# ClashLuke/LocAtE

Hardware: AMD Instinct MI355X
Metric: images/sec (G+D step) 64x64 bs=64 (higher is better)
Workload: dtype f32 (contractions fp32-faithful on the matrix cores: 2 x scaled fp16 operand pieces / 3 MFMAs per slice where the operand's largest magnitude comes with it, else 3 x bf16 pieces / 6 MFMAs; fp32 accumulate); 1 GPU; LocAtE G+D step, 64x64 RGB, batch 64 per GPU (the fp32 variant - the reference's own precision - of BASELINE.json configs[1]: 64x64 RGB bs 64), self/feature attention at 16x16 and 64x64, random-init weights; global_batch=64, image_size=64, parallelism=dp1, launch=hipGraph replay, G-step generator pass on a second stream

## Files before the change

locate_amd/build.py:

```python
import os
import shutil
import subprocess
import sys

CSRC = os.path.join(os.path.dirname(os.path.abspath(__file__)), "csrc")
LIB = os.path.join(CSRC, "liblocate_hip.so")
LIB_DBG = os.path.join(CSRC, "liblocate_hip_dbg.so")
DBG_SOURCES = ["conv.hip", "convwgrad.hip", "convwin.hip", "snapshot.hip"]
SOURCES = ["runtime.hip", "elementwise.hip", "norm.hip", "softmax.hip", "resample.hip", "spectral.hip", "conv.hip", "convpack.hip", "convwgrad.hip", "convwin.hip", "convfp8.hip",
           "grouped.hip", "nadam.hip", "loss.hip", "finalise.hip", "parallel.hip", "input.hip", "grid.hip", "swd.hip", "average.hip", "stats.hip", "guard.hip", "snapshot.hip", "digest.hip", "dynamics.hip", "neighbours.hip", "formats.hip", "spectrum.hip", "msssim.hip", "modes.hip"]
ARCH = "gfx950"


def _hipcc():
    for cand in (os.environ.get("HIPCC"), shutil.which("hipcc"), "/opt/rocm/bin/hipcc"):
        if cand and os.path.exists(cand):
            return cand
    raise RuntimeError("hipcc not found: the MI355X kernels cannot be built")


def _sources():
    return [s for s in SOURCES if os.path.exists(os.path.join(CSRC, s))]


def _headers():
    return [os.path.join(CSRC, h) for h in sorted(os.listdir(CSRC)) if h.endswith(".h")]


def needs_build():
    if not (os.path.exists(LIB) and os.path.exists(LIB_DBG)):
        return True
    t = min(os.path.getmtime(LIB), os.path.getmtime(LIB_DBG))
    deps = [os.path.join(CSRC, s) for s in _sources()] + _headers()
    return any(os.path.getmtime(d) > t for d in deps)


def build(force=False, verbose=True):
    if not force and not needs_build():
        return LIB
    hipcc = _hipcc()
    objs = []
    flags = ["--offload-arch=" + ARCH, "-O3", "-fPIC", "-std=c++17", "-fvisibility=hidden", "-Wall", "-Wno-unused-function",
             "-I", CSRC]
    procs = []
    hdr_time = max(os.path.getmtime(h) for h in _headers())
    for src in _sources():
        path = os.path.join(CSRC, src)
        obj = os.path.join(CSRC, src.replace(".hip", ".o"))
        objs.append(obj)
        if not force and os.path.exists(obj) and os.path.getmtime(obj) > max(os.path.getmtime(path), hdr_time):
            continue
        cmd = [hipcc] + flags + ["-c", path, "-o", obj]
        if verbose:
            print(" ".join(cmd), flush=True)
        procs.append((src, subprocess.Popen(cmd)))
    dbg_objs = list(objs)
    for src in DBG_SOURCES:
        path = os.path.join(CSRC, src)
        obj = os.path.join(CSRC, src.replace(".hip", "_dbg.o"))
        dbg_objs[dbg_objs.index(os.path.join(CSRC, src.replace(".hip", ".o")))] = obj
        if not force and os.path.exists(obj) and os.path.getmtime(obj) > max(os.path.getmtime(path), hdr_time):
            continue
        cmd = [hipcc] + flags + ["-DLOCATE_DEBUG_KNOBS", "-c", path, "-o", obj]
        if verbose:
            print(" ".join(cmd), flush=True)
        procs.append((src + " (debug)", subprocess.Popen(cmd)))
    failed = [src for src, p in procs if p.wait() != 0]
    if failed:
        raise RuntimeError("hipcc failed on " + ", ".join(failed))
    cmd = [hipcc, "--offload-arch=" + ARCH, "-shared", "-fPIC", "-o", LIB] + objs
    if verbose:
        print(" ".join(cmd), flush=True)
    subprocess.check_call(cmd)
    subprocess.check_call([hipcc, "--offload-arch=" + ARCH, "-shared", "-fPIC", "-o", LIB_DBG] + dbg_objs)
    return LIB


if __name__ == "__main__":
    build(force="--force" in sys.argv)
    print(LIB)
```

locate_amd/csrc/conv.hip:

```cpp
#include "igemm.h"

template <int WGM, int WGN, int TM, int TN>
__global__ void __launch_bounds__(256) conv_igemm_kernel(const IgParams p) {
    constexpr int BK = IG_BK;
    constexpr int BM = WGM * TM * 32;
    constexpr int BN = WGN * TN * 32;
    constexpr int KPT = BK * BN / 256;
    constexpr int A_F4 = BK * BM / 4;
    constexpr int A_PT = (A_F4 + 255) / 256;
    static_assert(WGM * WGN == 4, "four waves");
    static_assert(BN % 64 == 0 && KPT == 8, "one 8-row group of the offset table per thread and step");
    static_assert(BK <= IG_TAIL, "panel tail shorter than the prefetch distance (one stage beyond the last)");

    __shared__ __attribute__((aligned(16))) float As[2][BK][BM];
    __shared__ __attribute__((aligned(16))) float Bs[2][BK][BN];

    int bx, by, bz;
    xcd_tile(bx, by, bz, p.tile_nphase);
    const int zphase = bz / p.ksplit, zsplit = bz - zphase * p.ksplit;
    const IgPhase& ph = p.ph[zphase];
    const int N = p.B * ph.QH * ph.QW;
    const int n0 = bx * BN;
    const int m0 = by * BM;
    if (n0 >= N) return;
// ... 462 lines not shown
    const float sc = p.scale ? p.scale[(p.scale_bg ? b / p.scale_bg : 0) * p.scale_stride] : 1.0f;
    float* op = p.out + (long long)b * p.out_bs + q;
    if (p.act_out == nullptr && p.mul_pre == nullptr) {
#pragma unroll
        for (int m = 0; m < MT; ++m) {
            if (m < p.M && live) {
                const float bv = p.bias ? p.bias[m] : 0.0f;
                const float v0 = fmaf(acc[m][0], sc, bv), v1 = fmaf(acc[m][PX - 1], sc, bv);
                if (PX == 2) *reinterpret_cast<float2*>(op + (long long)m * HW) = make_float2(v0, v1);
                else op[(long long)m * HW] = v0;
            }
        }
        return;
    }
    float am = 0.0f;
    const float* zp = p.mul_pre ? p.mul_pre + (long long)b * p.mul_bs + q : nullptr;
    float* ap = p.act_out ? p.act_out + (long long)b * p.act_bs + q : nullptr;
#pragma unroll
    for (int m = 0; m < MT; ++m) {
        if (m < p.M && live) {
            const float bv = p.bias ? p.bias[m] : 0.0f;
            float v0 = fmaf(acc[m][0], sc, bv), v1 = fmaf(acc[m][PX - 1], sc, bv);
            if (zp) {
                float z0, z1;
                if (PX == 2) { const float2 t = *reinterpret_cast<const float2*>(zp + (long long)m * HW); z0 = t.x; z1 = t.y; }
                else { z0 = zp[(long long)m * HW]; z1 = z0; }
                v0 = roottanh_grad_f(z0, v0); v1 = roottanh_grad_f(z1, v1);
                am = fmaxf(am, fmaxf(fabsf(v0), fabsf(v1)));
            }
            if (PX == 2) *reinterpret_cast<float2*>(op + (long long)m * HW) = make_float2(v0, v1);
            else op[(long long)m * HW] = v0;
            if (ap) {
                const float a0 = roottanh_f(v0), a1 = roottanh_f(v1);
                if (PX == 2) *reinterpret_cast<float2*>(ap + (long long)m * HW) = make_float2(a0, a1);
                else ap[(long long)m * HW] = a0;
                am = fmaxf(am, fmaxf(fabsf(a0), fabsf(a1)));
            }
        }
    }
    if (p.out_absmax) absmax_publish_wave(am, p.out_absmax);
}


#define SK_NT 4
#define SK_RC 32
#define SK_WAVES 8

__global__ void __launch_bounds__(64 * SK_WAVES) skinny_rows_kernel(const IgParams p) {
    const IgPhase& ph = p.ph[0];
    const int R = ph.K, J = p.M, N = p.B, ld = ph.ld;
    const int lane = threadIdx.x & 63, wid = __builtin_amdgcn_readfirstlane((int)threadIdx.x >> 6);
    const int j = blockIdx.x * 64 + lane;
    const int n0 = blockIdx.y * SK_NT;
    const bool jok = j < ld;
    const float* __restrict__ P = ph.wp + (jok ? j : 0);
    const float* __restrict__ in = p.in;
    float acc[SK_NT];
#pragma unroll
    for (int t = 0; t < SK_NT; ++t) acc[t] = 0.0f;
    const int nchunk = (R + SK_RC - 1) / SK_RC;
    float cur[SK_RC], nxt[SK_RC];
    if (wid < nchunk) {
#pragma unroll
        for (int i = 0; i < SK_RC; ++i) cur[i] = P[(long long)(wid * SK_RC + i) * ld];
    }
    for (int c = wid; c < nchunk; c += SK_WAVES) {
        const int r0 = c * SK_RC;
        if (c + SK_WAVES < nchunk) {
#pragma unroll
            for (int i = 0; i < SK_RC; ++i) nxt[i] = P[(long long)(r0 + SK_WAVES * SK_RC + i) * ld];
        }
        if (r0 + SK_RC <= R) {
#pragma unroll
            for (int t = 0; t < SK_NT; ++t) {
                if (n0 + t < N) {
                    const float* __restrict__ xr = in + (long long)(n0 + t) * p.in_bs + r0;
#pragma unroll
                    for (int i = 0; i < SK_RC; ++i) acc[t] = fmaf(xr[i], cur[i], acc[t]);
                }
            }
        } else {
#pragma unroll
            for (int t = 0; t < SK_NT; ++t) {
                if (n0 + t < N) {
                    const float* __restrict__ xr = in + (long long)(n0 + t) * p.in_bs + r0;
#pragma unroll
                    for (int i = 0; i < SK_RC; ++i) {
                        const float xv = r0 + i < R ? xr[i] : 0.0f;
                        acc[t] = fmaf(xv, cur[i], acc[t]);
                    }
                }
            }
        }
#pragma unroll
        for (int i = 0; i < SK_RC; ++i) cur[i] = nxt[i];
    }
    __shared__ float red[SK_WAVES][SK_NT][64];
#pragma unroll
    for (int t = 0; t < SK_NT; ++t) red[wid][t][lane] = acc[t];
    __syncthreads();
    if (wid < SK_NT) {
        const int n = n0 + wid;
        float am = 0.0f;
        if (n < N && j < J) {
            float s = red[0][wid][lane];
#pragma unroll
            for (int w = 1; w < SK_WAVES; ++w) s += red[w][wid][lane];
            const float sc = p.scale ? p.scale[(p.scale_bg ? n / p.scale_bg : 0) * p.scale_stride] : 1.0f;
            float v = fmaf(s, sc, p.bias ? p.bias[j] : 0.0f);
            if (p.mul_pre) { v = roottanh_grad_f(p.mul_pre[(long long)n * p.mul_bs + j], v); am = fabsf(v); }
            p.out[(long long)n * p.out_bs + j] = v;
            if (p.act_out) { const float a = roottanh_f(v); p.act_out[(long long)n * p.act_bs + j] = a; am = fabsf(a); }
        }
        if (p.out_absmax) absmax_publish_wave(am, p.out_absmax);
        if (p.lat && blockIdx.x == 0 && n < N)
            for (int c = lane; c < p.lat_z; c += 64) p.act_out[(long long)n * p.act_bs - p.lat_z + c] = p.lat[(long long)n * p.lat_bs + c];
    }
}

static bool skinny_ok(const IgParams& p) {
    if (p.nphase != 1 || path_disabled("skinny")) return false;
    const IgPhase& ph = p.ph[0];
    return ph.T == 1 && p.H == 1 && p.W == 1 && p.OH == 1 && p.OW == 1 && ph.dy0 == 0 && ph.dx0 == 0 && ph.K >= 1;
}

static void launch_skinny(const IgParams& p, hipStream_t st) {
    skinny_rows_kernel<<<dim3((p.M + 63) / 64, (p.B + SK_NT - 1) / SK_NT), 64 * SK_WAVES, 0, st>>>(p);
}

static bool pointwise_ok(const IgParams& p) {
    if (p.nphase != 1 || path_disabled("pointwise")) return false;
    const IgPhase& ph = p.ph[0];
    const int HW = p.H * p.W;
    return ph.T == 1 && p.istride == 1 && p.ostep == 1 && ph.dy0 == 0 && ph.dx0 == 0 && p.H == p.OH && p.W == p.OW &&
           ph.K >= 1 && ph.K <= 64 && p.M <= 64 && ph.ld >= ((p.M + 15) / 16) * 16 && (HW & 1) == 0 && (p.in_bs & 1) == 0 &&
           (p.out_bs & 1) == 0 && (reinterpret_cast<uintptr_t>(p.in) & 7) == 0 && (reinterpret_cast<uintptr_t>(p.out) & 7) == 0 &&
           (long long)p.B * HW >= 131072 &&
           (!p.act_out || ((p.act_bs & 1) == 0 && (reinterpret_cast<uintptr_t>(p.act_out) & 7) == 0)) &&
           (!p.mul_pre || ((p.mul_bs & 1) == 0 && (reinterpret_cast<uintptr_t>(p.mul_pre) & 7) == 0));
}

template <int PX>
static void launch_pointwise_px(const IgParams& p, hipStream_t st) {
    const long long npx = (long long)p.B * p.H * p.W / PX;
    const int blocks = (int)((npx + 255) / 256);
    const int mt = (p.M + 15) / 16;
    if (mt == 1) conv_pointwise_kernel<16, PX><<<blocks, 256, 0, st>>>(p);
    else if (mt == 2) conv_pointwise_kernel<32, PX><<<blocks, 256, 0, st>>>(p);
    else if (mt == 3) conv_pointwise_kernel<48, PX><<<blocks, 256, 0, st>>>(p);
    else conv_pointwise_kernel<64, PX><<<blocks, 256, 0, st>>>(p);
}

static void launch_pointwise(const IgParams& p, hipStream_t st) {
    if ((long long)p.B * p.H * p.W >= (long long)knob_int("LOCATE_PX2_MIN", 2 * 256 * 1024)) launch_pointwise_px<2>(p, st);
    else launch_pointwise_px<1>(p, st);
}

static int igemm_bm(int M, int nmax, int nphase) {
    if (M % 192 == 0 && M >= 192 && !path_disabled("tall") && !path_disabled("bx6")) {
        const long long tiles = (long long)((nmax + 127) / 128) * (M / 192) * nphase;
        if (tiles >= 512) return 192;
    }
    return pick_bm(M);
}

static int igemm_ksplit(int M, int nmax, int nphase, int min_kpad) {
    const int bm = igemm_bm(M, nmax, nphase);
    const long long tiles = (long long)((nmax + 127) / 128) * ((M + bm - 1) / bm) * nphase;
    const int slots = bm == 192 ? 512 : 768;
    if (tiles >= slots || (tiles >= 512 && tiles % 256 == 0)) return 1;
    const int steps = min_kpad / IG_BK;
    long long want = (slots + tiles - 1) / tiles;
    const int min_steps = (long long)M * nmax <= (1 << 16) ? 2 : 8;
    if (steps < 8) return 1;
    const int max_split = steps / min_steps > 0 ? steps / min_steps : 1;
    if (want > max_split) want = max_split;
    if (want > 64) want = 64;
    if (want > knob_int("LOCATE_KS_MAX", 64)) want = knob_int("LOCATE_KS_MAX", 64);
    return want < 1 ? 1 : (int)want;
}

#define IG_MAX_COUNTERS 1024
struct SplitPlan {
    int ksplit, combine, gx, gy;
    size_t slab_floats;
};

static SplitPlan igemm_split_plan(const IgParams& p, int nmax, bool have_counters) {
    SplitPlan sp;
    const int bm = igemm_bm(p.M, nmax, p.nphase);
    int min_kpad = 1 << 30;
    for (int i = 0; i < p.nphase; ++i) min_kpad = p.ph[i].Kpad < min_kpad ? p.ph[i].Kpad : min_kpad;
    int ks = igemm_ksplit(p.M, nmax, p.nphase, min_kpad);
    if (ks > min_kpad / IG_BK) ks = min_kpad / IG_BK;
    if (ks < 1) ks = 1;
    sp.ksplit = ks;
    sp.gx = (nmax + 127) / 128;
    sp.gy = (p.M + bm - 1) / bm;
    const long long ntiles = (long long)sp.gx * sp.gy * p.nphase;
    const long long tile_floats = (long long)bm * 128;
    const long long legacy = ks > 1 ? (long long)ks * p.B * p.M * p.OH * p.OW : 0;
    const long long fused = ks > 1 ? (long long)ks * ntiles * tile_floats : 0;
    sp.combine = have_counters && ks > 1 && (long long)ks * tile_floats * 4 <= (512 << 10) && ntiles <= IG_MAX_COUNTERS &&
                 fused * 4 < (1ll << 31) && (p.precision == 1 || !path_disabled("bx6")) && !path_disabled("combine");
    sp.slab_floats = (size_t)(sp.combine ? fused : legacy);
    return sp;
}

void launch_slab_reduce(const IgParams& p, hipStream_t st) {
    igemm_slab_reduce_kernel<<<stream_grid(p.slab_stride, 256), 256, 0, st>>>(p.slab, p.out, p.bias, p.scale, p.scale_bg, p.scale_stride, p.B, p.M, p.OH * p.OW,
                                                                              p.out_bs, p.slab_stride, p.ksplit, p.act_out, p.act_bs, p.mul_pre, p.mul_bs, p.out_absmax);
}

template <int NP>
static void launch_bx6(const IgParams& p, dim3 grid, int bm, bool w8, hipStream_t st) {
    if (w8) {
        if (bm == 128) conv_igemm_bx6_kernel<2, 4, 2, 1, NP, 8><<<grid, 512, 0, st>>>(p);
        else conv_igemm_bx6_kernel<2, 4, 1, 1, NP, 8><<<grid, 512, 0, st>>>(p);
        return;
    }
    with_tile<true>(bm, [&](auto t) { using T = decltype(t); conv_igemm_bx6_kernel<T::wgm, T::wgn, T::tm, T::tn, NP><<<grid, 256, 0, st>>>(p); });
}

static int launch_igemm(IgParams& p, int nmax, void* slab_ws, unsigned* counters, hipStream_t st, const char* who) {
    p.tile_nphase = (path_disabled("phasefast") || (long long)p.OH * p.OW < 1024) ? 1 : p.nphase;
    if (p.win) return launch_win_igemm(p, nmax, slab_ws, counters, st, who);
    if (skinny_ok(p)) {
        p.ksplit = 1;
        launch_skinny(p, st);
        LOCATE_LAUNCH_CHECK(who);
        return LOCATE_OK;
    }
    if (pointwise_ok(p)) {
        p.ksplit = 1;
        launch_pointwise(p, st);
        LOCATE_LAUNCH_CHECK(who);
        return LOCATE_OK;
    }
    const int bm = igemm_bm(p.M, nmax, p.nphase);
    const SplitPlan sp = igemm_split_plan(p, nmax, counters != nullptr);
    p.ksplit = sp.ksplit;
    p.combine = sp.combine;
    p.counters = counters;
    p.slab = static_cast<float*>(slab_ws);
    p.slab_stride = (long long)p.B * p.M * p.OH * p.OW;
    dim3 grid(sp.gx, sp.gy, p.nphase * p.ksplit);
    for (int i = 0; i < p.nphase; ++i)
        LOCATE_REQUIRE(round_up(p.M, bm) <= p.ph[i].ld, "%s: tile height %d does not divide the panel width %d", who, bm, p.ph[i].ld);
    if (p.precision == 3) {
        launch_fp8_igemm(p, grid, bm, st);
        LOCATE_LAUNCH_CHECK(who);
        if (p.ksplit > 1 && !p.combine) {
            LOCATE_REQUIRE(p.slab_stride < (1ll << 31), "%s: split-K output of %lld elements exceeds the 32-bit index range", who, p.slab_stride);
            launch_slab_reduce(p, st);
            LOCATE_LAUNCH_CHECK(who);
        }
        return LOCATE_OK;
    }
    const bool w8 = !path_disabled("w8") && !path_disabled("bx6") && (bm == 128 || bm == 64) &&
                    (long long)grid.x * grid.y * grid.z <= knob_int("LOCATE_W8_MAX", 320);
    if (p.precision == 2) LOCATE_REQUIRE(!path_disabled("bx6"), "%s: fp16 pieces need the bf16/fp16 MFMA kernels", who);
    if (p.precision == 1) launch_bx6<1>(p, grid, bm, w8, st);
    else if (p.precision == 2) launch_bx6<2>(p, grid, bm, w8, st);
    else if (!path_disabled("bx6")) launch_bx6<3>(p, grid, bm, w8, st);
    else with_tile<false>(bm, [&](auto t) { using T = decltype(t); conv_igemm_kernel<T::wgm, T::wgn, T::tm, T::tn><<<grid, 256, 0, st>>>(p); });
    LOCATE_LAUNCH_CHECK(who);
    if (p.ksplit > 1 && !p.combine) {
        const long long total = p.slab_stride;
        LOCATE_REQUIRE(total < (1ll << 31), "%s: split-K output of %lld elements exceeds the 32-bit index range", who, total);
        launch_slab_reduce(p, st);
        LOCATE_LAUNCH_CHECK(who);
    }
    return LOCATE_OK;
}

static size_t slab_floats(const IgParams& p, int nmax) {
    if (p.win) return win_slab_floats(p, nmax);
    if (skinny_ok(p)) return 0;
    const size_t a = igemm_split_plan(p, nmax, false).slab_floats, b = igemm_split_plan(p, nmax, true).slab_floats;
    return a > b ? a : b;
}

static void useful_taps(int in, int out, int k, int s, int pad, int* lo, int* n) {
    if (path_disabled("taps")) { *lo = 0; *n = k; return; }
    int first = -1, last = -1;
    for (int t = 0; t < k; ++t) {
        bool any = false;
        for (int o = 0; o < out && !any; ++o) {
            const int i = o * s - pad + t;
            any = i >= 0 && i < in;
        }
        if (any) { if (first < 0) first = t; last = t; }
    }
    if (first < 0) { first = 0; last = 0; }
    *lo = first; *n = last - first + 1;
}
static void useful_phase_taps(int Q, int out, int d0, int T, int* lo, int* n) {
    if (path_disabled("taps")) { *lo = 0; *n = T > 0 ? T : 1; return; }
    int first = T > 0 ? d0 - out + 1 : 0, last = d0 + Q - 1;
    if (first < 0) first = 0;
    if (last > T - 1) last = T - 1;
    if (first > last) { first = 0; last = 0; }
    *lo = first; *n = last - first + 1;
}

static void phase_taps(int parity, int pad, int K, int s, int* k0, int* d0, int* T) {
// ... 375 lines not shown
```

locate_amd/csrc/igemm.h:

```cpp
#pragma once
#include "common.h"
#include <cstdlib>
#include <cstring>
#include <stdlib.h>
#include <type_traits>

#ifdef LOCATE_DEBUG_KNOBS
static bool path_disabled(const char* name) {
    static const char* env = getenv("LOCATE_DISABLE");
    return env != nullptr && strstr(env, name) != nullptr;
}
static int knob_int(const char* name, int fallback) {
    const char* v = getenv(name);
    return v != nullptr ? atoi(v) : fallback;
}
#else
static constexpr bool path_disabled(const char*) { return false; }
static constexpr int knob_int(const char*, int fallback) { return fallback; }
#endif

typedef float f32x16 __attribute__((ext_vector_type(16)));

#define IG_BK 16
#define IG_KPAD 32
// ... 67 lines not shown
    const unsigned* wmax;
    int direct;
    int keep_f32;
    int win, Tp, urows, wmax_single;
};

#define PACK_MAX_TAPS 32
struct PackBatch {
    PackArgs ph[4];
};
struct PackJob {
    PackBatch batch;
    int nphase, kind;
    int gx, gy;
    int block_start, pad;
};
PackJob make_pack_job(const PackBatch& b, int nphase);
int launch_pack(const PackBatch& b, int nphase, hipStream_t st, const char* who);

#define PANEL_HDR 4
static inline size_t panel_floats(int rows, int ld, int fmt) {
    if (fmt == 2) return (size_t)rows * ld + rows + rows / 4 + PANEL_HDR + (size_t)rows * ld / 4;
    return (size_t)rows * ld + rows + rows / 4 + (fmt ? PANEL_HDR + (size_t)rows * ld / 2 * 2 : (size_t)rows * ld / 2 * 3);
}
static inline size_t panel_split_offset(int rows, int ld) { return (size_t)rows * ld + rows + rows / 4; }
__device__ __forceinline__ size_t panel_split_offset_dev(int rows, int ld) { return (size_t)rows * ld + rows + rows / 4; }

__host__ __device__ __forceinline__ int scale_exp_below(int top, unsigned bits, unsigned grown) {
    const unsigned field = (bits >> 23) & 0xffu;
    if (grown == 0u ? field - 1u >= 254u : field == 255u) return 0;
    const int k = top - ((int)(field + grown) - 127);
    return k > 126 ? 126 : (k < -126 ? -126 : k);
}
__host__ __device__ __forceinline__ int f16_scale_exp(unsigned bits, unsigned grown = 0u) { return scale_exp_below(14, bits, grown); }
__host__ __device__ __forceinline__ int f8_scale_exp(unsigned bits, unsigned grown = 0u) { return scale_exp_below(7, bits, grown); }
__device__ __forceinline__ float pow2f(int k) { return __uint_as_float((unsigned)(k + 127) << 23); }
__device__ __forceinline__ void unscale_pair(int ka, int kb, float& u1, float& u2) {
    const int t = -(ka + kb), h = t >> 1;
    u1 = pow2f(h);
    u2 = pow2f(t - h);
}

typedef __bf16 bf16x8 __attribute__((ext_vector_type(8)));

__device__ __forceinline__ void split3_bf16x8(const float (&v)[8], bf16x8& h, bf16x8& m, bf16x8& l) {
#pragma unroll
    for (int j = 0; j < 8; ++j) {
        h[j] = (__bf16)v[j];
        const float r1 = v[j] - (float)h[j];
        m[j] = (__bf16)r1;
        l[j] = (__bf16)(r1 - (float)m[j]);
    }
}

__device__ __forceinline__ void split3_trunc_pair(float v0, float v1, unsigned& h, unsigned& m, unsigned& l) {
    const unsigned u0 = __builtin_bit_cast(unsigned, v0), u1 = __builtin_bit_cast(unsigned, v1);
    const float r0 = v0 - __builtin_bit_cast(float, u0 & 0xffff0000u), r1 = v1 - __builtin_bit_cast(float, u1 & 0xffff0000u);
    const unsigned q0 = __builtin_bit_cast(unsigned, r0), q1 = __builtin_bit_cast(unsigned, r1);
    const float l0 = r0 - __builtin_bit_cast(float, q0 & 0xffff0000u), l1 = r1 - __builtin_bit_cast(float, q1 & 0xffff0000u);
    h = __builtin_amdgcn_perm(u1, u0, 0x07060302u);
    m = __builtin_amdgcn_perm(q1, q0, 0x07060302u);
    l = __builtin_amdgcn_perm(__builtin_bit_cast(unsigned, l1), __builtin_bit_cast(unsigned, l0), 0x07060302u);
}

__device__ __forceinline__ unsigned round_bf16_pair(float v0, float v1) {
    typedef __bf16 bf16x2_t __attribute__((ext_vector_type(2)));
    bf16x2_t r;
    r[0] = (__bf16)v0;
    r[1] = (__bf16)v1;
    return *reinterpret_cast<unsigned*>(&r);
}

__device__ __forceinline__ void split3_trunc_x8(const float (&v)[8], uint4& h, uint4& m, uint4& l) {
    split3_trunc_pair(v[0], v[1], h.x, m.x, l.x);
    split3_trunc_pair(v[2], v[3], h.y, m.y, l.y);
    split3_trunc_pair(v[4], v[5], h.z, m.z, l.z);
    split3_trunc_pair(v[6], v[7], h.w, m.w, l.w);
}

typedef _Float16 f16x8 __attribute__((ext_vector_type(8)));

__device__ __forceinline__ void split2_f16x8(const float (&v)[8], float sc, uint4& h, uint4& l) {
    f16x8 hh, ll;
#pragma unroll
    for (int j = 0; j < 8; ++j) {
        const float x = v[j] * sc;
        hh[j] = (_Float16)x;
        ll[j] = (_Float16)(x - (float)hh[j]);
    }
    h = *reinterpret_cast<uint4*>(&hh);
    l = *reinterpret_cast<uint4*>(&ll);
}

__device__ __forceinline__ void split2_f16_pair(float v0, float v1, unsigned& h, unsigned& l) {
    typedef _Float16 f16x2 __attribute__((ext_vector_type(2)));
    f16x2 hh, ll;
    hh[0] = (_Float16)v0; hh[1] = (_Float16)v1;
    ll[0] = (_Float16)(v0 - (float)hh[0]); ll[1] = (_Float16)(v1 - (float)hh[1]);
    h = *reinterpret_cast<unsigned*>(&hh);
    l = *reinterpret_cast<unsigned*>(&ll);
}

struct IgPhase {
    const float* wp;
    const int* koff;
    const unsigned char* ktap;
    const uint4* w3;
    const unsigned* a_absmax;
    long long w3_plane;
    int K, Kpad, ld, T;
    int dmin;
    int oy0, ox0, QH, QW;
    int TW, tw_magic;
    int dy0, dys, dx0, dxs;
    int win_Tp, win_NG, win_TR, win_NI, win_WR;
    unsigned win_wrw_mul;
    int win_wrw_s1, win_wrw_s2;
    int tapc[32] __attribute__((aligned(32)));
};

struct IgParams {
    const float* in;
    float* out;
    const float* bias;
    const float* scale;
    int scale_bg;
    int scale_stride;
    long long in_bs, out_bs;
    unsigned in_bytes;
    int B, C, H, W;
    int M, OH, OW;
    int istride, ostep, nphase;
    int ksplit;
    float* slab;
    long long slab_stride;
    int precision;
    const unsigned* b_absmax;
    float* act_out = nullptr;
    long long act_bs = 0;
    const float* lat = nullptr;
    long long lat_bs = 0;
    int lat_z = 0;
    const float* mul_pre = nullptr;
    long long mul_bs = 0;
    unsigned* out_absmax = nullptr;
    int combine;
    unsigned* counters;
    int tile_nphase;
    int win;
    int win_dbg;
    int win_U, win_slotsp, win_bm, win_bn;
    IgPhase ph[4];
};

template <int WGM, int WGN, int TM, int TN>
__device__ __forceinline__ void igemm_col_scales(const IgParams& p, const IgPhase& ph, float (&col_scale)[TN], int N, int n0,
                                                 int wn, int lane) {
    const int lcol = lane & 31;
#pragma unroll
    for (int j = 0; j < TN; ++j) {
        const int nj = n0 + (wn * TN + j) * 32 + lcol;
        const int nn = nj < N ? nj : 0;
        const int b = nn / (ph.QH * ph.QW);
        col_scale[j] = p.scale ? p.scale[(p.scale_bg ? b / p.scale_bg : 0) * p.scale_stride] : 1.0f;
    }
}

template <int WGM, int WGN, int TM, int TN>
__device__ __forceinline__ void igemm_epilogue(const IgParams& p, const IgPhase& ph, f32x16 (&acc)[TM][TN],
                                               const float (&col_scale)[TN], int N, int n0, int m0, int zsplit, int wm,
                                               int wn, int lane, float* stage, bool split) {
    const int lrow = lane >> 5, lcol = lane & 31;
    const long long plane = (long long)p.OH * p.OW;
    const int iplane = (int)plane;
    if (stage != nullptr && p.nphase == 1 && p.ostep == 1 && iplane <= 16 && (iplane & (iplane - 1)) == 0 &&
        ph.QH * ph.QW == iplane) {
        const int lp = __ffs(iplane) - 1;
        const bool fused_s = !split && (p.act_out != nullptr || p.mul_pre != nullptr);
        float am_s = 0.0f;
        float* out_base = split ? p.slab + (long long)zsplit * p.slab_stride : p.out;
        const long long obs = split ? (long long)p.M * plane : p.out_bs;
#pragma unroll
        for (int i = 0; i < TM; ++i) {
            const int mt0 = m0 + (wm * TM + i) * 32;
            float bias_v[16];
#pragma unroll
            for (int r = 0; r < 16; ++r) {
                const int m = mt0 + (r & 3) + 8 * (r >> 2) + 4 * lrow;
                const bool use = p.bias != nullptr && !split && m < p.M;
                const float* bp = use ? p.bias + m : p.in;
                bias_v[r] = use ? *bp : 0.0f;
            }
#pragma unroll
            for (int j = 0; j < TN; ++j) {
                const int nt0 = n0 + (wn * TN + j) * 32;
#pragma unroll
                for (int r = 0; r < 16; ++r) {
                    const int ml = (r & 3) + 8 * (r >> 2) + 4 * lrow;
                    stage[lcol * 33 + ml] = split ? acc[i][j][r] : fmaf(acc[i][j][r], col_scale[j], bias_v[r]);
                }
                __builtin_amdgcn_fence(__ATOMIC_SEQ_CST, "wavefront");
                const int b0 = nt0 >> lp;
                if (!fused_s) {
#pragma unroll
                    for (int e = 0; e < 16; ++e) {
                        const int flat = e * 64 + lane;
                        const int bl = flat >> (5 + lp), rem = flat & ((32 << lp) - 1);
                        const int ml = rem >> lp, pix = rem & (iplane - 1);
                        const int nl = (bl << lp) + pix;
                        const float v = stage[nl * 33 + ml];
                        if (nt0 + nl < N && mt0 + ml < p.M) out_base[(long long)(b0 + bl) * obs + (long long)(mt0 + ml) * plane + pix] = v;
                    }
                } else if (WGM * WGN == 8 && TM * TN <= 2 && p.mul_pre != nullptr) {
                    __builtin_amdgcn_sched_barrier(0);
                    float z[16];
#pragma unroll
                    for (int e = 0; e < 16; ++e) {
                        const int flat = e * 64 + lane;
                        const int bl = flat >> (5 + lp), rem = flat & ((32 << lp) - 1);
                        const int ml = rem >> lp, pix = rem & (iplane - 1);
                        const int nl = (bl << lp) + pix;
                        const bool ok = nt0 + nl < N && mt0 + ml < p.M;
                        z[e] = ok ? p.mul_pre[(long long)(b0 + bl) * p.mul_bs + (long long)(mt0 + ml) * plane + pix] : 0.0f;
                    }
#pragma unroll
                    for (int e = 0; e < 16; ++e) {
                        const int flat = e * 64 + lane;
                        const int bl = flat >> (5 + lp), rem = flat & ((32 << lp) - 1);
                        const int ml = rem >> lp, pix = rem & (iplane - 1);
                        const int nl = (bl << lp) + pix;
                        if (nt0 + nl < N && mt0 + ml < p.M) {
                            const float v = roottanh_grad_f(z[e], stage[nl * 33 + ml]);
                            am_s = fmaxf(am_s, fabsf(v));
                            out_base[(long long)(b0 + bl) * obs + (long long)(mt0 + ml) * plane + pix] = v;
                        }
                    }
                    __builtin_amdgcn_sched_barrier(0);
                } else {
#pragma unroll 1
                    for (int e = 0; e < 16; ++e) {
                        const int flat = e * 64 + lane;
                        const int bl = flat >> (5 + lp), rem = flat & ((32 << lp) - 1);
                        const int ml = rem >> lp, pix = rem & (iplane - 1);
                        const int nl = (bl << lp) + pix;
                        float v = stage[nl * 33 + ml];
                        if (nt0 + nl < N && mt0 + ml < p.M) {
                            const long long rel = (long long)(mt0 + ml) * plane + pix;
                            if (p.mul_pre != nullptr) {
                                v = roottanh_grad_f(p.mul_pre[(long long)(b0 + bl) * p.mul_bs + rel], v);
                                am_s = fmaxf(am_s, fabsf(v));
                            }
                            out_base[(long long)(b0 + bl) * obs + rel] = v;
                            if (p.mul_pre == nullptr) {
                                const float a = roottanh_f(v);
                                p.act_out[(long long)(b0 + bl) * p.act_bs + rel] = a;
                                am_s = fmaxf(am_s, fabsf(a));
                            }
                        }
                    }
                }
                __builtin_amdgcn_fence(__ATOMIC_SEQ_CST, "wavefront");
            }
        }
        if (fused_s && p.out_absmax != nullptr) absmax_publish_wave(am_s, p.out_absmax);
        return;
    }
    const float* optr[TN];
    long long xoff[TN];
    const bool fused = !split && (p.act_out != nullptr || p.mul_pre != nullptr);
#pragma unroll
    for (int j = 0; j < TN; ++j) {
        const int nj = n0 + (wn * TN + j) * 32 + lcol;
        const int nn = nj < N ? nj : 0;
        const int qhw = ph.QH * ph.QW;
        const int b = nn / qhw, q = nn - b * qhw;
        const int qy = q / ph.QW, qx = q - qy * ph.QW;
        const long long pix = (long long)(ph.oy0 + qy * p.ostep) * p.OW + (ph.ox0 + qx * p.ostep);
        const float* o = split ? p.slab + (long long)zsplit * p.slab_stride + (long long)b * p.M * plane + pix
                               : p.out + (long long)b * p.out_bs + pix;
        optr[j] = nj < N ? o : nullptr;
        xoff[j] = (long long)b * ((p.mul_pre ? p.mul_bs : p.act_bs) - p.out_bs);
    }
    float am = 0.0f;
#pragma unroll
    for (int i = 0; i < TM; ++i) {
        float bias_v[16];
#pragma unroll
        for (int r = 0; r < 16; ++r) {
            const int m = m0 + (wm * TM + i) * 32 + (r & 3) + 8 * (r >> 2) + 4 * lrow;
            const bool use = p.bias != nullptr && !split && m < p.M;
            const float* bp = use ? p.bias + m : p.in;
            bias_v[r] = use ? *bp : 0.0f;
        }
#pragma unroll
        for (int j = 0; j < TN; ++j) {
            float* o = const_cast<float*>(optr[j]);
            if (o == nullptr) continue;
            if (!fused) {
#pragma unroll
                for (int r = 0; r < 16; ++r) {
                    const int m = m0 + (wm * TM + i) * 32 + (r & 3) + 8 * (r >> 2) + 4 * lrow;
                    if (m < p.M) o[(long long)m * plane] = split ? acc[i][j][r] : fmaf(acc[i][j][r], col_scale[j], bias_v[r]);
                }
            } else if (p.mul_pre != nullptr) {
                const float* pre = p.mul_pre + ((o - p.out) + xoff[j]);
#pragma unroll
// ... 115 lines not shown
```

Before: 7368 images/sec.

## Add MFMA-based persistent pointwise conv kernel with register-resident weights

Adds a new 1x1 (pointwise) convolution kernel that keeps the weights in registers and computes on fp32 32x32x2 MFMA instructions. It runs as a persistent grid capped at a per-CU block count, with a ring buffer that prefetches the next tile's input while the current tile computes. It can also fuse the roottanh activation, its gradient multiply and absmax publishing into the epilogue. It replaces the scalar pointwise kernel when shapes and alignment qualify, aiming to lift arithmetic throughput and hide load latency, at the cost of many templated variants and heavy register pressure.

```diff
diff --git a/locate_amd/build.py b/locate_amd/build.py
--- a/locate_amd/build.py
+++ b/locate_amd/build.py
@@ -7,7 +7,7 @@
 LIB = os.path.join(CSRC, "liblocate_hip.so")
 LIB_DBG = os.path.join(CSRC, "liblocate_hip_dbg.so")
 DBG_SOURCES = ["conv.hip", "convwgrad.hip", "convwin.hip", "snapshot.hip"]
-SOURCES = ["runtime.hip", "elementwise.hip", "norm.hip", "softmax.hip", "resample.hip", "spectral.hip", "conv.hip", "convpack.hip", "convwgrad.hip", "convwin.hip", "convfp8.hip",
+SOURCES = ["runtime.hip", "elementwise.hip", "norm.hip", "softmax.hip", "resample.hip", "spectral.hip", "conv.hip", "convpw.hip", "convpack.hip", "convwgrad.hip", "convwin.hip", "convfp8.hip",
            "grouped.hip", "nadam.hip", "loss.hip", "finalise.hip", "parallel.hip", "input.hip", "grid.hip", "swd.hip", "average.hip", "stats.hip", "guard.hip", "snapshot.hip", "digest.hip", "dynamics.hip", "neighbours.hip", "formats.hip", "spectrum.hip", "msssim.hip", "modes.hip"]
 ARCH = "gfx950"
 
diff --git a/locate_amd/csrc/conv.hip b/locate_amd/csrc/conv.hip
--- a/locate_amd/csrc/conv.hip
+++ b/locate_amd/csrc/conv.hip
@@ -638,6 +638,7 @@
 }
 
 static void launch_pointwise(const IgParams& p, hipStream_t st) {
+    if (!path_disabled("pwmfma") && pointwise_mfma_ok(p)) { launch_pointwise_mfma(p, knob_int("LOCATE_PWM_BLOCKS", 0), st); return; }
     if ((long long)p.B * p.H * p.W >= (long long)knob_int("LOCATE_PX2_MIN", 2 * 256 * 1024)) launch_pointwise_px<2>(p, st);
     else launch_pointwise_px<1>(p, st);
 }
diff --git a/locate_amd/csrc/convpw.hip b/locate_amd/csrc/convpw.hip
--- /dev/null
+++ b/locate_amd/csrc/convpw.hip
@@ -0,0 +1,222 @@
+#include "igemm.h"
+
+#define PWM_CUS 256
+#define PWM_NTP 4
+
+template <int MT, int NQ, int RD, int WPS, bool FUSED>
+__global__ void __launch_bounds__(256, WPS) conv_pointwise_mfma_kernel(const IgParams p) {
+    constexpr int NTP = PWM_NTP, NJ = 2 * NQ;
+    static_assert(NJ % RD == 0, "the ring divides the tile");
+    const IgPhase& ph = p.ph[0];
+    const int lane = threadIdx.x & 63, c = lane & 31, h = lane >> 5;
+    const int HW = p.H * p.W, K = ph.K, ld = ph.ld, M = p.M;
+    const unsigned NP = (unsigned)p.B * (unsigned)HW;
+    const unsigned ntiles = (NP + 32 * NTP - 1) / (32 * NTP);
+    const unsigned nwaves = gridDim.x * 4;
+    unsigned tile = blockIdx.x * 4 + (unsigned)__builtin_amdgcn_readfirstlane((int)threadIdx.x >> 6);
+    const DivU32 dhw((unsigned)HW);
+
+    float w[MT][NJ];
+    {
+        const float* __restrict__ wp = ph.wp;
+#pragma unroll
+        for (int j = 0; j < NJ; ++j)
+#pragma unroll
+            for (int mt = 0; mt < MT; ++mt) {
+                const int m = mt * 32 + c;
+                w[mt][j] = wp[(long long)(2 * j + h) * ld + (m < ld ? m : 0)];
+                if (m >= ld) w[mt][j] = 0.0f;
+            }
+    }
+    const int bias_bits = __float_as_int((p.bias != nullptr && lane < M) ? p.bias[lane] : 0.0f);
+
+    auto coords = [&](unsigned t, unsigned& b, unsigned& q) -> bool {
+        const unsigned n = t * (32 * NTP) + NTP * (unsigned)c;
+        const bool live = n < NP;
+        dhw.divmod(live ? n : 0u, b, q);
+        return live;
+    };
+    auto load_scale = [&](unsigned b) -> float {
+        const float* sp = p.scale ? p.scale : ph.wp;
+        const float v = sp[p.scale ? (p.scale_bg ? (int)b / p.scale_bg : 0) * p.scale_stride : 0];
+        return p.scale ? v : 1.0f;
+    };
+    int hv = h;
+    auto load_pair = [&](const float* ip, int j) -> float4 {
+        const int k = min(2 * j + hv, K - 1);
+        return *reinterpret_cast<const float4*>(ip + k * HW);
+    };
+    auto bias_of = [&](int m0) -> float {
+        const int lo = __builtin_amdgcn_readlane(bias_bits, m0), hi = __builtin_amdgcn_readlane(bias_bits, m0 + 4);
+        return __int_as_float(hv ? hi : lo);
+    };
+
+    float4 x[RD];
+    unsigned b = 0, q = 0;
+    bool live = false;
+    float sc = 1.0f, am = 0.0f;
+    const float* ip = p.in;
+
+    auto step = [&](auto prefetch) {
+        constexpr bool PREFETCH = decltype(prefetch)::value;
+        asm volatile("" : "+v"(hv));
+        unsigned nb = 0, nqx = 0;
+        bool nlive = false;
+        float nsc = 1.0f;
+        const float* nip = nullptr;
+        if constexpr (PREFETCH) {
+            nlive = coords(tile + nwaves, nb, nqx);
+            nsc = load_scale(nb);
+            nip = p.in + (long long)nb * p.in_bs + nqx;
+        }
+        f32x16 acc[MT][NTP];
+#pragma unroll
+        for (int mt = 0; mt < MT; ++mt)
+#pragma unroll
+            for (int t = 0; t < NTP; ++t)
+#pragma unroll
+                for (int r = 0; r < 16; ++r) acc[mt][t][r] = 0.0f;
+#pragma unroll
+        for (int j = 0; j < NJ; ++j) {
+            const float4 xv = x[j % RD];
+#pragma unroll
+            for (int mt = 0; mt < MT; ++mt) {
+                acc[mt][0] = __builtin_amdgcn_mfma_f32_32x32x2f32(w[mt][j], xv.x, acc[mt][0], 0, 0, 0);
+                acc[mt][1] = __builtin_amdgcn_mfma_f32_32x32x2f32(w[mt][j], xv.y, acc[mt][1], 0, 0, 0);
+                acc[mt][2] = __builtin_amdgcn_mfma_f32_32x32x2f32(w[mt][j], xv.z, acc[mt][2], 0, 0, 0);
+                acc[mt][3] = __builtin_amdgcn_mfma_f32_32x32x2f32(w[mt][j], xv.w, acc[mt][3], 0, 0, 0);
+            }
+            if (j + RD < NJ) { x[j % RD] = load_pair(ip, j + RD); __builtin_amdgcn_sched_barrier(0); }
+            else if constexpr (PREFETCH) { x[j % RD] = load_pair(nip, j + RD - NJ); __builtin_amdgcn_sched_barrier(0); }
+        }
+        float* op = p.out + (long long)b * p.out_bs + q;
+        if constexpr (!FUSED && PREFETCH) {
+            float4 v = make_float4(0.0f, 0.0f, 0.0f, 0.0f);
+            int row = 0;
+#pragma unroll
+            for (int mt = 0; mt < MT; ++mt)
+#pragma unroll
+                for (int r = 0; r < 16; ++r) {
+                    const int m0 = mt * 32 + (r & 3) + 8 * (r >> 2), m = m0 + 4 * hv;
+                    const float bv = bias_of(m0);
+                    const float4 vr = make_float4(fmaf(acc[mt][0][r], sc, bv), fmaf(acc[mt][1][r], sc, bv), fmaf(acc[mt][2][r], sc, bv),
+                                                  fmaf(acc[mt][3][r], sc, bv));
+                    if (m0 < 4 || m < M) { v = vr; row = m; }
+                    *reinterpret_cast<float4*>(op + row * HW) = v;
+                }
+        } else if constexpr (!FUSED) {
+#pragma unroll
+            for (int mt = 0; mt < MT; ++mt)
+#pragma unroll
+                for (int r = 0; r < 16; ++r) {
+                    const int m0 = mt * 32 + (r & 3) + 8 * (r >> 2), m = m0 + 4 * hv;
+                    const float bv = bias_of(m0);
+                    if ((m < M) & live)
+                        *reinterpret_cast<float4*>(op + m * HW) = make_float4(fmaf(acc[mt][0][r], sc, bv), fmaf(acc[mt][1][r], sc, bv),
+                                                                              fmaf(acc[mt][2][r], sc, bv), fmaf(acc[mt][3][r], sc, bv));
+                }
+        } else {
+            const float* zp = p.mul_pre ? p.mul_pre + (long long)b * p.mul_bs + q : nullptr;
+            float* ap = p.act_out ? p.act_out + (long long)b * p.act_bs + q : nullptr;
+            constexpr int ZB = 4;
+#pragma unroll
+            for (int mt = 0; mt < MT; ++mt) {
+                float4 zb[ZB];
+#pragma unroll
+                for (int r = 0; r < 16; ++r) {
+                    const int m0 = mt * 32 + (r & 3) + 8 * (r >> 2), m = m0 + 4 * hv;
+                    if (r % ZB == 0 && zp) {
+#pragma unroll
+                        for (int i = 0; i < ZB; ++i) {
+                            const int mi = mt * 32 + ((r + i) & 3) + 8 * ((r + i) >> 2) + 4 * hv;
+                            zb[i] = *reinterpret_cast<const float4*>(zp + (mi < M ? mi : 0) * HW);
+                        }
+                    }
+                    const float bv = bias_of(m0);
+                    if ((m < M) & live) {
+                        float v[NTP] = {fmaf(acc[mt][0][r], sc, bv), fmaf(acc[mt][1][r], sc, bv), fmaf(acc[mt][2][r], sc, bv),
+                                        fmaf(acc[mt][3][r], sc, bv)};
+                        if (zp) {
+                            const float4 z4 = zb[r % ZB];
+                            const float z[NTP] = {z4.x, z4.y, z4.z, z4.w};
+#pragma unroll
+                            for (int t = 0; t < NTP; ++t) { v[t] = roottanh_grad_f(z[t], v[t]); am = fmaxf(am, fabsf(v[t])); }
+                        }
+                        *reinterpret_cast<float4*>(op + m * HW) = make_float4(v[0], v[1], v[2], v[3]);
+                        if (ap) {
+                            float a[NTP];
+#pragma unroll
+                            for (int t = 0; t < NTP; ++t) { a[t] = roottanh_f(v[t]); am = fmaxf(am, fabsf(a[t])); }
+                            *reinterpret_cast<float4*>(ap + m * HW) = make_float4(a[0], a[1], a[2], a[3]);
+                        }
+                    }
+                }
+            }
+        }
+        b = nb; q = nqx; live = nlive; sc = nsc; ip = nip;
+    };
+
+    if (tile < ntiles) {
+        live = coords(tile, b, q);
+        sc = load_scale(b);
+        ip = p.in + (long long)b * p.in_bs + q;
+#pragma unroll
+        for (int j = 0; j < RD; ++j) x[j] = load_pair(ip, j);
+        if (tile + nwaves < ntiles) {
+            step(std::true_type{});
+            for (tile += nwaves; tile + nwaves < ntiles; tile += nwaves) step(std::true_type{});
+            step(std::false_type{});
+        } else {
+            step(std::false_type{});
+        }
+    }
+    if (FUSED && p.out_absmax) absmax_publish_wave(am, p.out_absmax);
+}
+
+bool pointwise_mfma_ok(const IgParams& p) {
+    const long long HW = (long long)p.H * p.W;
+    auto al = [](const void* q, long long bs) { return (reinterpret_cast<uintptr_t>(q) & 15) == 0 && (bs & 3) == 0; };
+    const bool fused = p.act_out != nullptr || p.mul_pre != nullptr;
+    return (long long)p.B * HW < (1ll << 31) - 32 * PWM_NTP && HW < (1 << 24) && (HW & 3) == 0 && p.M > 16 && p.M <= 64 &&
+           p.ph[0].K >= 1 && p.ph[0].K <= 64 && al(p.in, p.in_bs) && al(p.out, p.out_bs) && (!p.act_out || al(p.act_out, p.act_bs)) &&
+           (!p.mul_pre || al(p.mul_pre, p.mul_bs)) && (!fused || p.M <= 32) && !(p.ph[0].K <= 4 && p.M > 32);
+}
+
+template <int MT, int NQ, bool FUSED>
+constexpr int pwm_regs(int rd) { return 64 * MT + 2 * NQ * MT + 4 * rd + (FUSED ? 60 : 28); }
+template <int MT, int NQ, bool FUSED>
+constexpr int pwm_ring() {
+    for (int rd = 2 * NQ; rd > 1; --rd)
+        if ((2 * NQ) % rd == 0 && pwm_regs<MT, NQ, FUSED>(rd) <= 232) return rd;
+    return 1;
+}
+template <int MT, int NQ, bool FUSED>
+constexpr int pwm_wps() {
+    const int regs = pwm_regs<MT, NQ, FUSED>(pwm_ring<MT, NQ, FUSED>());
+    return regs <= 120 ? 4 : (regs <= 160 ? 3 : 2);
+}
+
+template <int MT, int NQ, bool FUSED>
+static void launch_pwm_form(const IgParams& p, int blocks_per_cu, hipStream_t st) {
+    constexpr int RD = pwm_ring<MT, NQ, FUSED>(), WPS = pwm_wps<MT, NQ, FUSED>();
+    const long long ntiles = ((long long)p.B * p.H * p.W + 32 * PWM_NTP - 1) / (32 * PWM_NTP);
+    const long long blocks = (ntiles + 3) / 4;
+    const int cap = PWM_CUS * (blocks_per_cu > 0 ? blocks_per_cu : 1);
+    conv_pointwise_mfma_kernel<MT, NQ, RD, WPS, FUSED><<<(int)(blocks < cap ? blocks : cap), 256, 0, st>>>(p);
+}
+
+template <int MT, int NQ>
+static void launch_pwm(const IgParams& p, int nq, int blocks_per_cu, hipStream_t st) {
+    if (nq == NQ) {
+        if (p.act_out == nullptr && p.mul_pre == nullptr) launch_pwm_form<MT, NQ, false>(p, blocks_per_cu, st);
+        else if constexpr (MT == 1) launch_pwm_form<MT, NQ, true>(p, blocks_per_cu, st);
+    } else if constexpr (NQ < 16) {
+        launch_pwm<MT, NQ + 1>(p, nq, blocks_per_cu, st);
+    }
+}
+
+void launch_pointwise_mfma(const IgParams& p, int blocks_per_cu, hipStream_t st) {
+    const int nq = (p.ph[0].K + 3) / 4;
+    if (p.M <= 32) launch_pwm<1, 1>(p, nq, blocks_per_cu, st);
+    else launch_pwm<2, 1>(p, nq, blocks_per_cu, st);
+}
diff --git a/locate_amd/csrc/igemm.h b/locate_amd/csrc/igemm.h
--- a/locate_amd/csrc/igemm.h
+++ b/locate_amd/csrc/igemm.h
@@ -243,6 +243,9 @@
     int win_U, win_slotsp, win_bm, win_bn;
     IgPhase ph[4];
 };
+
+bool pointwise_mfma_ok(const IgParams& p);
+void launch_pointwise_mfma(const IgParams& p, int blocks_per_cu, hipStream_t st);
 
 template <int WGM, int WGN, int TM, int TN>
 __device__ __forceinline__ void igemm_col_scales(const IgParams& p, const IgPhase& ph, float (&col_scale)[TN], int N, int n0,
```

New measurement: 7357 images/sec. No clear change (-0.2%).
